# zraorg/ZRA

Measured on AMD Instinct MI355X. Metric: compress + RA-decompress GiB/s, 16 GiB @ 64 KiB frames, 1/2/4/8 MI355X, higher is better.
Workload: dtype u8

## Files before the change

zra_amd/csrc/zra_decode.hip:

```cpp
#include "zra_dev.h"
#include "zra_kernels.h"

using namespace zra_dev;

namespace {

constexpr int DEC_THREADS = 64;
constexpr int BATCH = 64;
#ifndef ZRA_XWIN
#define ZRA_XWIN 4032
#endif
constexpr u32 XPRE = 64, XWIN = ZRA_XWIN;
constexpr u32 BLOCK_MAX = 128u << 10;

__constant__ u32 c_ll_base[36] = {0,1,2,3,4,5,6,7,8,9,10,11,12,13,14,15,16,18,20,22,24,28,32,40,48,64,128,256,512,1024,2048,4096,8192,16384,32768,65536};
__constant__ u8 c_ll_bits[36] = {0,0,0,0,0,0,0,0,0,0,0,0,0,0,0,0,1,1,1,1,2,2,3,3,4,6,7,8,9,10,11,12,13,14,15,16};
__constant__ u32 c_ml_base[53] = {3,4,5,6,7,8,9,10,11,12,13,14,15,16,17,18,19,20,21,22,23,24,25,26,27,28,29,30,31,32,33,34,
                                  35,37,39,41,43,47,51,59,67,83,99,131,259,515,1027,2051,4099,8195,16387,32771,65539};
__constant__ u8 c_ml_bits[53] = {0,0,0,0,0,0,0,0,0,0,0,0,0,0,0,0,0,0,0,0,0,0,0,0,0,0,0,0,0,0,0,0,
                                 1,1,1,1,2,2,3,3,4,4,5,7,8,9,10,11,12,13,14,15,16};
__constant__ short c_ll_defnorm[36] = {4,3,2,2,2,2,2,2,2,2,2,2,2,1,1,1,2,2,2,2,2,2,2,2,2,3,2,1,1,1,1,1,-1,-1,-1,-1};
__constant__ short c_ml_defnorm[53] = {1,4,3,2,2,2,2,2,2,1,1,1,1,1,1,1,1,1,1,1,1,1,1,1,1,1,1,1,1,1,1,1,
                                       1,1,1,1,1,1,1,1,1,1,1,1,1,1,-1,-1,-1,-1,-1,-1,-1};
__constant__ short c_of_defnorm[29] = {1,1,1,1,1,1,2,2,2,1,1,1,1,1,1,1,1,1,1,1,1,1,1,1,-1,-1,-1,-1,-1};
// ... 976 lines not shown
        packed |= (e & 0xFF) << (8 * k);
        hb.skip((int)(e >> 8));
      }
      pk[g] = packed;
    }
    st128(o + i, pk[0], pk[1], pk[2], pk[3]);
  }
  for (; i + 4 <= count; i += 4) {
    hb.ensure(4 * mb);
    u32 packed = 0;
#pragma unroll
    for (int k = 0; k < 4; k++) {
      u32 e = tab[hb.peek(mb)];
      packed |= (e & 0xFF) << (8 * k);
      hb.skip((int)(e >> 8));
    }
    st32(o + i, packed);
  }
  for (; i < count; i++) { hb.ensure(mb); u32 e = tab[hb.peek(mb)]; o[i] = (u8)e; hb.skip((int)(e >> 8)); }
}

__device__ __forceinline__ bool huf_decode_stream(const ZraDecodeArgs& a, ZraDecFrame* const F, const u32 j, const u16* const tab, const u8* const w1,
                                                  const u32 strm, const u8* const lim) {
  const u32 nStreams = F->litStreams, regen = F->litRegen;
  const u32 seg = nStreams == 1 ? regen : (regen + 3) / 4;
  const u32 myLen = nStreams == 1 ? regen : (strm < 3 ? seg : regen - 3 * seg);
  u8* o = a.lits + F->litBase + (size_t)strm * seg;
  const u8* const blk = a.body + a.frameOff[frame_of(a, j) * a.offStride] + F->bpos;
  const u8* const sb = blk + F->streamOff[strm]; const u32 sl = F->streamLen[strm];
  const int mb = (int)F->hufMaxBits;
#ifndef ZRA_HUF_READER_AHEAD
#define ZRA_HUF_READER_AHEAD 1
#endif
#if ZRA_HUF_READER_AHEAD
  BitRS hb;
#else
  BitR hb;
#endif
  bool bad = hb.init(sb, sl, lim) != 0;
  if (!bad) {
    u32 i = 0;
    if (mb < 12) {
      huf_x1_emit(hb, tab, mb, o, myLen);
      i = myLen;
    } else {
      for (; i < myLen; i++) { hb.ensure(12); const u32 e = huf_lookup12(tab, w1, hb.peek(12), 12); o[i] = (u8)e; hb.skip((int)(e >> 8)); }
    }
    if (hb.pos != 0) bad = true;
  }
  if (bad && F->hufX2) bad = !huf_stream_x2(tab, w1, (u32)mb, sb, sl, lim, o, myLen);
  return !bad;
}

__device__ __forceinline__ bool huf_decode_wave(const ZraDecodeArgs& a, const ZraDecFrame* const F, const u32 j, const u16* const tab, const int lane, const u8* const lim) {
  const u32 nStreams = F->litStreams, regen = F->litRegen;
  const int mb = (int)F->hufMaxBits;
  if (mb >= 12 || regen < 64) return false;
  const u32 L = nStreams == 1 ? 64u : 16u;
  const u32 strm = nStreams == 1 ? 0u : (u32)lane >> 4, t = (u32)lane & (L - 1);
  const u32 seg = nStreams == 1 ? regen : (regen + 3) / 4;
  const u32 myLen = nStreams == 1 ? regen : (strm < 3 ? seg : regen - 3 * seg);
  const u8* const blk = a.body + a.frameOff[frame_of(a, j) * a.offStride] + F->bpos;
  const u8* const sb = blk + F->streamOff[strm]; const u32 sl = F->streamLen[strm];
  const u32 last = sl ? (u32)sb[sl - 1] : 0u;
  if (__ballot(last == 0)) return false;
  const u32 P = (sl - 1) * 8 + hb32(last);
  const u32 C = max((P + L - 1) / L, 128u);
  const bool active = t * C < P;
  const i32 lower = (t + 1) * C >= P ? 0 : (i32)(P - (t + 1) * C);
  i32 start = (i32)(P - t * C), end = 0;
  u32 n = 0;
  bool dirty = active;
  BitRS hb;
  i32 prevStart = start;
  for (int it = 0; it < 6 && __ballot(dirty); it++) {
    if (dirty) {
      bool merged = false;
      if (it) {
        BitRS ho;
        hb.init_at(sb, lim, start); ho.init_at(sb, lim, prevStart);
        u32 ka = 0, kb = 0;
        for (int k = 0; k < 96; k++) {
          if (hb.pos == ho.pos) { merged = true; break; }
          if (hb.pos <= lower || ho.pos <= lower) break;
          if (hb.pos > ho.pos) { hb.ensure(mb); const u32 e = tab[hb.peek(mb)]; hb.skip((int)(e >> 8)); ka++; }
          else { ho.ensure(mb); const u32 e = tab[ho.peek(mb)]; ho.skip((int)(e >> 8)); kb++; }
        }
        if (merged) n = ka + (n - kb);
      }
      if (!merged) {
        hb.init_at(sb, lim, start); n = 0;
        while (hb.pos > lower) {
          hb.ensure(4 * mb);
#pragma unroll
          for (int k = 0; k < 4; k++) if (hb.pos > lower) { const u32 e = tab[hb.peek(mb)]; hb.skip((int)(e >> 8)); n++; }
        }
        end = hb.pos;
      }
    }
    const i32 handed = (i32)__shfl_up(end, 1, 64);
    const i32 ns = t == 0 ? (i32)P : handed;
    prevStart = start;
    dirty = active && ns != start;
    start = ns;
#ifdef ZRA_SMALL_PROFILE
    { const u64 dm = __ballot(dirty); if (lane == 0) atomicAdd(&zra_small_prof[16 + it], (u64)__popcll(dm)); }
#endif
  }
#ifdef ZRA_SMALL_PROFILE
  if (lane == 0) atomicAdd(&zra_small_prof[6], 1ull);
  if (__ballot(dirty) && lane == 0) atomicAdd(&zra_small_prof[7], 1ull);
#endif
  if (__ballot(dirty)) return false;
  u32 incl = active ? n : 0u;
  if (L == 64) incl = dpp_scan_add(incl);
  else {
    incl += (u32)__builtin_amdgcn_update_dpp(0, (int)incl, 0x111, 0xF, 0xF, true);
    incl += (u32)__builtin_amdgcn_update_dpp(0, (int)incl, 0x112, 0xF, 0xF, true);
    incl += (u32)__builtin_amdgcn_update_dpp(0, (int)incl, 0x114, 0xF, 0xF, true);
    incl += (u32)__builtin_amdgcn_update_dpp(0, (int)incl, 0x118, 0xF, 0xF, true);
  }
  const u32 total = (u32)__shfl((int)incl, (int)(((u32)lane & ~(L - 1)) + L - 1), 64);
  if (__ballot(total != myLen || (active && lower == 0 && end != 0))) return false;
  if (active && n) {
    hb.init_at(sb, lim, start);
    huf_x1_emit(hb, tab, mb, a.lits + F->litBase + (size_t)strm * seg + (incl - n), n);
  }
  return true;
}
}

extern "C" __global__ void __launch_bounds__(DEC_THREADS)
zra_dec_huf_kernel(ZraDecodeArgs a) {
  __shared__ HufShared S;
  const int lane = threadIdx.x;
  const u32 nJobs = a.counters[ZRA_DC_NHUF];
  const u8* const lim = a.body + a.bodySize;
  for (;;) {
    wsync();
    if (lane == 0) S.base = atomicAdd(&a.counters[ZRA_DC_QHUF], (u32)HUF_FRAMES);
    wsync();
    const u32 base = S.base;
    if (base >= nJobs) return;
    const u32 nHere = min((u32)HUF_FRAMES, nJobs - base);
    for (u32 s = 0; s < nHere; s++) huf_build_table(&a.frames[a.hufJobs[base + s]], S.tab[s], S.w1[s], lane);
    wsync();
    u32 doneMask = 0;
    for (u32 s = 0; s < nHere; s++) {
      const u32 j = a.hufJobs[base + s];
      if (huf_decode_wave(a, &a.frames[j], j, S.tab[s], lane, lim)) doneMask |= 1u << s;
    }
    const u32 slot = (u32)lane >> 2, strm = (u32)lane & 3;
    if (slot < nHere && !((doneMask >> slot) & 1u)) {
      const u32 j = a.hufJobs[base + slot];
      ZraDecFrame* const F = &a.frames[j];
      if (strm < F->litStreams && !huf_decode_stream(a, F, j, S.tab[slot], S.w1[slot], strm, lim)) F->hufErr = 1;
    }
  }
}

namespace {

constexpr u32 CHAIN_RING = 128, CHAIN_RING_WORDS = (CHAIN_RING + 16) / 4;
static_assert(CHAIN_RING_WORDS == ZRA_CHAIN_RING_WORDS, "ring size: zra_kernels.h");
__device__ __attribute__((noinline)) uint4 chain_ld128_tail(const u8* p, const u8* lim) {
  u32 w[4] = {0, 0, 0, 0};
  for (u32 k = 0; k < 16; k++) if (p + k < lim) w[k >> 2] |= (u32)p[k] << (8 * (k & 3));
  return make_uint4(w[0], w[1], w[2], w[3]);
}
template <bool RING>
struct ZdsT {
  u64 c; u32 bc; u32 ptr;
  const u8* base;
  u8* ring; u32 rLo; const u8* lim; uint4 pf; u32 pfState, pfAge;
  enum : int { UNFINISHED = 0, ENDOFBUFFER = 1, COMPLETED = 2, OVERFLOW = 3 };
  __device__ __forceinline__ uint4 ld16(const u8* p) const {
    if (p + 16 <= lim) { const u128_u q = *(const u128_u*)p; return make_uint4(q.a, q.b, q.c, q.d); }
    return chain_ld128_tail(p, lim);
  }
  __device__ __forceinline__ void ring_write(u32 off, uint4 q) {
    const u32 o = off & (CHAIN_RING - 1);
    lds_st128(ring + o, q);
    if (o == 0) lds_st64(ring + CHAIN_RING, (u64)q.x | ((u64)q.y << 32));
  }
  __device__ __forceinline__ void ring_resync(u32 p) {
    const u32 pc = p & ~15u, lo = pc >= 48 ? pc - 48 : 0u;
    uint4 q[5];
#pragma unroll
    for (u32 k = 0; k < 5; k++) q[k] = ld16(base + lo + 16 * k);
#pragma unroll
    for (u32 k = 0; k < 5; k++) ring_write(lo + 16 * k, q[k]);
    rLo = lo; pfState = 0;
  }
  __device__ __forceinline__ void ring_advance() {
    if (pfState) {
      if (++pfAge >= 2 && ptr + 8 + 16 <= rLo + CHAIN_RING) { ring_write(rLo - 16, pf); rLo -= 16; pfState = 0; }
    } else if (rLo >= 16 && ptr < rLo + 64) { pf = ld16(base + rLo - 16); pfState = 1; pfAge = 0; }
  }
  __device__ __forceinline__ u64 fetch(u32 p) {
    if (RING) return *(const zra_lds_u64u_t*)(ring + (p & (CHAIN_RING - 1)));
    return ld64(base + p);
  }
  __device__ __forceinline__ void ring_guard() { if (rLo && ptr < rLo + 16) ring_resync(ptr); }
// ... 890 lines not shown
```

zra_amd/csrc/zra_dev.h:

```cpp
#pragma once
#include <hip/hip_runtime.h>
#include <stdint.h>

namespace zra_dev {

typedef uint8_t u8;
typedef uint16_t u16;
typedef uint32_t u32;
typedef uint64_t u64;
typedef int32_t i32;

enum : u32 {
  ZE_OK = 0, ZE_GENERIC = 1, ZE_PREFIX_UNKNOWN = 10, ZE_FRAMEPARAM_UNSUPPORTED = 14, ZE_WINDOW_TOO_LARGE = 16,
  ZE_CORRUPTION = 20, ZE_CHECKSUM_WRONG = 22, ZE_DICT_CORRUPTED = 30, ZE_DICT_WRONG = 32, ZE_PARAM_UNSUPPORTED = 40,
  ZE_DSTSIZE_TOOSMALL = 70, ZE_SRCSIZE_WRONG = 72,
};

constexpr int WAVE = 64;

__host__ __device__ __forceinline__ u64 frame_expect(u64 i, u64 frameSize, u64 total) {
  const u64 o = i * frameSize;
  return o >= total ? 0 : (total - o < frameSize ? total - o : frameSize);
}

__device__ __forceinline__ u32 hb32(u32 x) { return 31u - (u32)__builtin_clz(x); }
__device__ __forceinline__ int lane_id() { return (int)(threadIdx.x & 63); }

typedef u16 __attribute__((aligned(1))) u16_u;
typedef u32 __attribute__((aligned(1))) u32_u;
typedef u64 __attribute__((aligned(1))) u64_u;
__device__ __forceinline__ u32 ld16(const u8* p) { return *(const u16_u*)p; }
__device__ __forceinline__ u32 ld24(const u8* p) { return (u32)p[0] | ((u32)p[1] << 8) | ((u32)p[2] << 16); }
__device__ __forceinline__ u32 ld32(const u8* p) { return *(const u32_u*)p; }
__device__ __forceinline__ u64 ld64(const u8* p) { return *(const u64_u*)p; }
__device__ __forceinline__ u64 ld64_safe(const u8* p, const u8* end) {
  if (p + 8 <= end) return ld64(p);
  u64 v = 0;
  for (int i = 0; i < 8; i++) if (p + i < end) v |= (u64)p[i] << (8 * i);
  return v;
}
typedef __attribute__((address_space(3))) u64_u zra_lds_u64u_t;
typedef u32 zra_v4u32_t __attribute__((ext_vector_type(4)));
typedef __attribute__((address_space(3))) zra_v4u32_t zra_lds_v4u32_t;
typedef __attribute__((address_space(3))) u64 zra_lds_u64_t;
__device__ __forceinline__ void lds_st128(u8* p, uint4 q) { zra_v4u32_t v = {q.x, q.y, q.z, q.w}; *(zra_lds_v4u32_t*)p = v; }
__device__ __forceinline__ void lds_st64(u8* p, u64 v) { *(zra_lds_u64_t*)p = v; }
__device__ __forceinline__ void st32(u8* p, u32 v) { *(u32_u*)p = v; }
__device__ __forceinline__ void st64(u8* p, u64 v) { *(u64_u*)p = v; }
__device__ __forceinline__ void copy_bytes(u8* dst, const u8* src, u32 n, int t, int nthreads) {
  u32 n8 = n >> 3;
  for (u32 i = t; i < n8; i += nthreads) st64(dst + 8 * i, ld64(src + 8 * i));
  for (u32 i = (n8 << 3) + t; i < n; i += nthreads) dst[i] = src[i];
}
__device__ __forceinline__ void copy_slice(u8* dst, const u8* src, u32 n, int lane) {
  if ((((uintptr_t)dst ^ (uintptr_t)src) & 15u) || n < 64) { copy_bytes(dst, src, n, lane, 64); return; }
  const u32 head = (u32)((16u - ((uintptr_t)dst & 15u)) & 15u);
  if ((u32)lane < head) dst[lane] = src[lane];
  const u32 n16 = (n - head) >> 4;
  const uint4* s4 = (const uint4*)(src + head);
  uint4* d4 = (uint4*)(dst + head);
  for (u32 i = lane; i < n16; i += 64) d4[i] = s4[i];
  for (u32 i = head + (n16 << 4) + lane; i < n; i += 64) dst[i] = src[i];
}
__device__ __forceinline__ u64 seek_entry(const u8* table, u64 f) { const u8* e = table + (size_t)f * 5; return (u64)ld32(e) | ((u64)e[4] << 32); }
struct Slice { u32 tuple; u64 frame; u32 inFrame; u32 len; u64 user; };
__device__ __forceinline__ Slice slice_of(const u64* q, u32 nq, u64 s, u64 fs) {
  u32 lo = 0, hi = nq - 1;
  while (lo < hi) {
    const u32 mid = lo + (hi - lo + 1) / 2;
    if (q[4 * (size_t)mid + 3] <= s) lo = mid; else hi = mid - 1;
  }
  const u64 off = q[4 * (size_t)lo], size = q[4 * (size_t)lo + 1], k = s - q[4 * (size_t)lo + 3];
  const u64 f0 = off / fs, head = off - f0 * fs;
  Slice r;
  r.tuple = lo; r.frame = f0 + k;
  r.inFrame = k ? 0u : (u32)head;
  const u64 done = k ? (fs - head) + (k - 1) * fs : 0;
  r.len = (u32)min<u64>(fs - r.inFrame, size - done);
  r.user = q[4 * (size_t)lo + 2] + done;
  return r;
}
struct __attribute__((packed, aligned(1))) u128_u { u32 a, b, c, d; };
__device__ __forceinline__ void st128(u8* p, u32 a, u32 b, u32 c, u32 d) { u128_u v; v.a = a; v.b = b; v.c = c; v.d = d; *(u128_u*)p = v; }

__device__ __forceinline__ u32 wave_incl_scan(u32 v) {
  int l = lane_id();
#pragma unroll
  for (int d = 1; d < 64; d <<= 1) {
    u32 t = __shfl_up(v, d, 64);
    if (l >= d) v += t;
  }
  return v;
}
__device__ __forceinline__ u32 wave_sum(u32 v) {
#pragma unroll
  for (int d = 32; d > 0; d >>= 1) v += __shfl_xor(v, d, 64);
  return v;
}
__device__ __forceinline__ u32 wave_max(u32 v) {
#pragma unroll
  for (int d = 32; d > 0; d >>= 1) { u32 t = __shfl_xor(v, d, 64); v = t > v ? t : v; }
  return v;
}

struct BitR {
  const u8* base;
  const u8* lim;
  i32 pos;
  i32 wlo;
  u64 w;
  __device__ __forceinline__ void reload() {
    i32 byteIdx = ((pos + 7) >> 3) - 8;
    if (byteIdx >= 0) { w = ld64_safe(base + byteIdx, lim); wlo = byteIdx * 8; }
    else {
      i32 sh = -byteIdx * 8;
      w = sh >= 64 ? 0 : (ld64_safe(base, lim) << sh);
      wlo = byteIdx * 8;
    }
  }
  __device__ __forceinline__ int init(const u8* b, u32 n, const u8* bufLim) {
    base = b; lim = bufLim;
    if (n == 0) return 1;
    u32 last = b[n - 1];
    if (last == 0) return 1;
    pos = (i32)(n - 1) * 8 + (i32)hb32(last);
    reload();
    return 0;
  }
  __device__ __forceinline__ void ensure(int nb) { if (pos - wlo < nb) reload(); }
  __device__ __forceinline__ u32 peek(int nb) const {
    return (u32)((w >> (pos - nb - wlo)) & ((1ull << nb) - 1));
  }
  __device__ __forceinline__ void skip(int nb) { pos -= nb; }
  __device__ __forceinline__ u32 read(int nb) {
    if (nb == 0) return 0;
    ensure(nb);
    u32 v = peek(nb);
    pos -= nb;
    return v;
  }
};

struct BitRS {
  const u8* base; const u8* lim;
  i32 pos, wlo; u64 w;
  i32 gtop;
  u64 g0, g1, g2;
  __device__ __forceinline__ u64 grid(i32 idx) const {
    if (idx >= 0) return ld64_safe(base + idx, lim);
    if (idx <= -8) return 0;
    return ld64_safe(base, lim) << (u32)(-idx * 8);
  }
  __device__ __forceinline__ void reload() {
    const i32 byteIdx = ((pos + 7) >> 3) - 8;
    while (byteIdx <= gtop - 8) { g0 = g1; g1 = g2; gtop -= 8; g2 = grid(gtop - 16); }
    const u32 d = (u32)(gtop - byteIdx);
    w = d ? ((g0 << (8 * d)) | (g1 >> (64 - 8 * d))) : g0;
    wlo = byteIdx * 8;
  }
  __device__ __forceinline__ int init(const u8* b, u32 n, const u8* bufLim) {
    base = b; lim = bufLim;
    if (n == 0) return 1;
    u32 last = b[n - 1];
    if (last == 0) return 1;
    pos = (i32)(n - 1) * 8 + (i32)hb32(last);
    gtop = ((pos + 7) >> 3) - 8;
    g0 = grid(gtop); g1 = grid(gtop - 8); g2 = grid(gtop - 16);
    w = g0; wlo = gtop * 8;
    return 0;
  }
  __device__ __forceinline__ void init_at(const u8* b, const u8* bufLim, i32 p) {
    base = b; lim = bufLim; pos = p;
    gtop = ((pos + 7) >> 3) - 8;
    g0 = grid(gtop); g1 = grid(gtop - 8); g2 = grid(gtop - 16);
    w = g0; wlo = gtop * 8;
  }
  __device__ __forceinline__ void ensure(int nb) { if (pos - wlo < nb) reload(); }
  __device__ __forceinline__ u32 peek(int nb) const { return (u32)((w >> (pos - nb - wlo)) & ((1ull << nb) - 1)); }
  __device__ __forceinline__ void skip(int nb) { pos -= nb; }
};


constexpr u64 XP1 = 11400714785074694791ULL, XP2 = 14029467366897019727ULL, XP3 = 1609587929392839161ULL,
              XP4 = 9650029242287828579ULL, XP5 = 2870177450012600261ULL;
__device__ __forceinline__ u64 rotl64(u64 x, int r) { return (x << r) | (x >> (64 - r)); }
__device__ __forceinline__ u64 xxround(u64 acc, u64 x) { return rotl64(acc + x * XP2, 31) * XP1; }
__device__ __forceinline__ u64 xxmerge(u64 h, u64 v) { return (h ^ xxround(0, v)) * XP1 + XP4; }


__device__ inline u64 zra_xxh64_quad(const u8* p, u32 n, int j) {
  u64 v = j == 0 ? XP1 + XP2 : j == 1 ? XP2 : j == 2 ? 0 : (0 - XP1);
  const u32 stripes = n >> 5;
  const u8* q = p + 8 * j;
  u32 s = 0;
  for (; s + 8 <= stripes; s += 8) {
    u64 x[8];
#pragma unroll
    for (int k = 0; k < 8; k++) x[k] = ld64(q + 32 * (size_t)(s + k));
#pragma unroll
    for (int k = 0; k < 8; k++) v = xxround(v, x[k]);
  }
  for (; s < stripes; s++) v = xxround(v, ld64(q + 32 * (size_t)s));
  const int base = (threadIdx.x & 63) & ~3;
  u64 v1 = __shfl(v, base + 0, 64), v2 = __shfl(v, base + 1, 64), v3 = __shfl(v, base + 2, 64), v4 = __shfl(v, base + 3, 64);
  u64 h;
  if (n >= 32) {
    h = rotl64(v1, 1) + rotl64(v2, 7) + rotl64(v3, 12) + rotl64(v4, 18);
    h = xxmerge(h, v1); h = xxmerge(h, v2); h = xxmerge(h, v3); h = xxmerge(h, v4);
  } else h = XP5;
  h += (u64)n;
  if (j == 0) {
    const u8* t = p + ((size_t)stripes << 5); u32 rem = n & 31;
    while (rem >= 8) { h = rotl64(h ^ xxround(0, ld64(t)), 27) * XP1 + XP4; t += 8; rem -= 8; }
    if (rem >= 4) { h = rotl64(h ^ ((u64)ld32(t) * XP1), 23) * XP2 + XP3; t += 4; rem -= 4; }
    while (rem) { h = rotl64(h ^ ((u64)*t * XP5), 11) * XP1; t++; rem--; }
    h ^= h >> 33; h *= XP2; h ^= h >> 29; h *= XP3; h ^= h >> 32;
  }
  return h;
}

__device__ inline u64 zra_xxh64_quad_seed(const u8* p, u64 n, int j, u64 seed) {
  u64 v = seed + (j == 0 ? XP1 + XP2 : j == 1 ? XP2 : j == 2 ? 0 : (0 - XP1));
  const u64 stripes = n >> 5;
  const u8* q = p + 8 * j;
  u64 s = 0;
  for (; s + 8 <= stripes; s += 8) {
    u64 x[8];
#pragma unroll
    for (int k = 0; k < 8; k++) x[k] = ld64(q + 32 * (size_t)(s + k));
#pragma unroll
    for (int k = 0; k < 8; k++) v = xxround(v, x[k]);
  }
// ... 22 lines not shown
```

zra_amd/csrc/zra_engine.h:

```cpp
#pragma once
#include <hip/hip_runtime.h>
#include <cstdint>
#include <cstddef>
#include <vector>
#include "zra_kernels.h"
#include "zra_scan_plan.h"

namespace zra_eng {

struct Status { int zra; int zstd; };
enum : int { kSuccess = 0, kZStdError = 1, kVersionLow = 2, kHeaderInvalid = 3, kHeaderIncomplete = 4, kOutOfBounds = 5,
             kOutputTooSmall = 6, kCompressedTooLarge = 7, kFrameSizeMismatch = 8 };
inline Status ok() { return {kSuccess, 0}; }
inline Status zerr(int code) { return {kZStdError, (int)(int8_t)code}; }

struct DevBuf {
  void* p = nullptr; size_t cap = 0;
  bool reserve(size_t n);
  void release();
  template <typename T> T* as() const { return (T*)p; }
};

uint64_t scratch_bytes_in_use();

// ... 147 lines not shown
  void locate_records_stats(uint64_t out[8]) const { for (int i = 0; i < 8; i++) out[i] = lstats_[i]; }
  double locate_records_ms() const { return locateMs_; }
  Status read_records(const uint8_t* dArc, size_t arcSize, const uint64_t info6[6], const uint64_t* dIndex, size_t indexWords, const uint64_t* hNumbers, size_t n,
                      size_t stagingBytes, uint64_t* hRanges, uint8_t* dData, size_t dataCap, uint64_t* dataSize);
  void read_records_stats(uint64_t out[8]) const { for (int i = 0; i < 8; i++) out[i] = rstats_[i]; }
  double read_records_ms() const { return readMs_; }

  Status compress_host(const uint8_t* hIn, size_t n, uint8_t* hOut, size_t* outSize, int level, uint32_t frameSize, bool checksum);
  Status compress_frames_host(const uint8_t* hIn, size_t n, uint8_t* hBody, std::vector<uint64_t>& sizes, size_t* bodySize,
                              int level, uint32_t frameSize, bool checksum);
  Status decode_host(const uint8_t* hSpan, size_t spanSize, const std::vector<uint64_t>& starts, const std::vector<uint64_t>& ends,
                     uint32_t frameSize, uint64_t total, uint8_t* hOut, size_t skip, size_t size, bool wholeArchive = false);
  Status decode_host_pipelined(const uint8_t* hSpan, const std::vector<uint64_t>& starts, const std::vector<uint64_t>& ends,
                               uint32_t frameSize, uint64_t total, uint8_t* hOut, bool* fallBack);

  void set_ra_verify_whole_frames(bool on) { raVerifyWholeFrames_ = on; }
  bool ra_verify_whole_frames() const { return raVerifyWholeFrames_; }
  int device() const { return device_; }
  int num_cus() const { return numCUs_; }

 private:
  Engine() = default;
  int device_ = 0, numCUs_ = 0;
  hipStream_t stream_ = nullptr;
  hipEvent_t ev0_ = nullptr, ev1_ = nullptr, evWait_ = nullptr;
  double lastKernelMs_ = 0;
  std::vector<uint64_t> mfTele_;
  const uint64_t* mfTeleDev_ = nullptr;
  double kstats_[6] = {0, 0, 0, 0, 0, 0};
  double dstats_[8] = {0, 0, 0, 0, 0, 0, 0, 0};
  std::vector<hipEvent_t> stageEv_; size_t stageEvNext_ = 0;
  hipEvent_t stage_event();
  Status launch_stages(uint64_t nJobs, const struct ZraDecodeArgs& a, const struct ZraDecodeArgs& mid, uint32_t nFrames, bool blockPass, hipEvent_t se[5]);
  Status launch_chain(uint64_t nJobs, const struct ZraDecodeArgs& mid, hipEvent_t after);
  Status decode_sequential_tail(const struct ZraDecodeArgs& a, const uint64_t* dFrameOff, uint32_t offStride, const uint64_t* dOutOff, uint32_t first,
                                uint32_t nFrames, uint32_t maxFrameBytes, uint64_t seqTotal);
  Status upload_jobs(const std::vector<uint64_t>& frameOff, const std::vector<uint64_t>& outOff, const std::vector<uint32_t>& expect);
  Status read_fixed_header(const uint8_t* dArc, size_t arcSize, HeaderInfo* h);
  uint64_t* pinned_tuples(size_t nTuples);
  void reset_decode_stats() { kstats_[4] = kstats_[5] = 0; for (auto& d : dstats_) d = 0; }
  static float elapsed_ms(hipEvent_t e0, hipEvent_t e1) { float ms = 0; if (hipEventElapsedTime(&ms, e0, e1) != hipSuccess) { ms = 0; (void)hipGetLastError(); } return ms; }
  bool call_events() {
    for (auto& ev : evCall_) if (!ev && hipEventCreate(&ev) != hipSuccess) { ev = nullptr; (void)hipGetLastError(); return false; }
    return true;
  }
  void free_scratch();
  hipEvent_t evR_[17] = {nullptr};
  DevBuf decFrames_, decTables_, decLists_, decCounters_, decLits_, decSeqs_, roundN_;
  DevBuf decBlkRecs_, decBlkTables_, decBlkLists_;
  DevBuf raPlan_, raLimit_, raPieceBase_, raPieces_;
  uint8_t* pinSmall_ = nullptr;
  uint64_t* pinQ_ = nullptr; size_t pinQCap_ = 0;
  int decOccParse_ = 0, decOccExec_ = 0, decOccHuf_ = 0;
  bool raVerifyWholeFrames_ = false;
  DevBuf status_, produced_, frameMeta_, frameOff_, outOff_, expect_, result_, qmeta_;
  DevBuf stage_;
  struct EncCtx { DevBuf tables, seqs, lits, work, slots, misc, ck, sizes, rec; };
  EncCtx encCtx_[2];
  DevBuf encScan_;
  DevBuf mfFlags_;
  int lsAttr_ = 0;
  hipStream_t stream2_ = nullptr;
  bool decCountersClean_ = false;
  int chainLdsAttr_ = 0;
  hipStream_t pipeStreams_[2] = {nullptr, nullptr};
  std::vector<hipEvent_t> evPool_;
  DevBuf hostIn_, hostOut_, seqScratch_;
  uint64_t dbgSeqStride_ = 0; uint32_t dbgB_ = 0;
  uint64_t lastProducedTotal_ = ~0ull;
  void* encCounters_ = nullptr; size_t encCountersBytes_ = 0;
  int waitValueOk_ = 0;
  struct UpdScratch { DevBuf plan, packed, encSizes, frames, table, copies; } upd_;
  uint64_t ustats_[8] = {0, 0, 0, 0, 0, 0, 0, 0};
  hipEvent_t evCall_[2] = {nullptr, nullptr};
  double updStageMs_ = 0;
  struct VerifyScratch { DevBuf plan, faults; } vfy_;
  uint64_t vstats_[8] = {0, 0, 0, 0, 0, 0, 0, 0};
  struct ScanScratch { DevBuf tables, list; } scan_;
  uint64_t scanStats_[kScanCalls][8] = {};
  double scanMs_[kScanCalls] = {};
  struct CompareScratch { DevBuf flags, tables, list; } cmp_;
  uint64_t cstats_[8] = {0, 0, 0, 0, 0, 0, 0, 0}, cmpSizes_[2] = {0, 0};
  double compareMs_ = 0;
  uint64_t fstats_[8] = {0, 0, 0, 0, 0, 0, 0, 0};
  double diffMs_ = 0;
  struct SignScratch { DevBuf flags, dirty, tables, list; } sig_;
  uint64_t gstats_[8] = {0, 0, 0, 0, 0, 0, 0, 0}, hstats_[8] = {0, 0, 0, 0, 0, 0, 0, 0};
  double signMs_ = 0, sigDiffMs_ = 0;
  struct RecScratch { DevBuf tables, ranges; } rec_;
  uint64_t istats_[8] = {0, 0, 0, 0, 0, 0, 0, 0}, lstats_[8] = {0, 0, 0, 0, 0, 0, 0, 0}, rstats_[8] = {0, 0, 0, 0, 0, 0, 0, 0};
  double indexMs_ = 0, locateMs_ = 0, readMs_ = 0;
  friend struct EncodeImpl;
  friend struct UpdateImpl;
  friend struct VerifyImpl;
  friend struct ScanImpl;
  friend struct CompareImpl;
  friend struct DiffImpl;
  friend struct SignImpl;
  friend struct RecordsImpl;
  friend class ArchiveCache;
};

void search_launch_jobs(hipStream_t s, const uint8_t* table, uint64_t fs, uint64_t total, uint64_t first, uint32_t n, uint64_t* frameOff, uint64_t* outOff,
                        uint32_t* expect);
void search_launch_scan(hipStream_t s, const uint32_t* counts, uint32_t nItems, uint64_t* bases, const uint64_t* cntIn, uint64_t* cntOut);
void search_launch_carry(hipStream_t s, uint8_t* win, uint64_t L, uint32_t n);
// ... 5 lines not shown
```

zra_amd/csrc/zra_engine.hip:

```cpp
#include "zra_host.h"
#include "zra_dev.h"
#include "zra_format.h"
#include <algorithm>
#include <atomic>

extern "C" __global__ void zra_dec_parse_kernel(ZraDecodeArgs a);
extern "C" __global__ void zra_dec_huf_kernel(ZraDecodeArgs a);
extern "C" __global__ void zra_dec_chain_kernel(ZraDecodeArgs a);
extern "C" __global__ void zra_dec_chain_lds_kernel(ZraDecodeArgs a);
extern "C" __global__ void zra_dec_exec_kernel(ZraDecodeArgs a);
extern "C" __global__ void zra_dec_parse_all_kernel(ZraDecodeArgs a);
extern "C" __global__ void zra_dec_exec_all_kernel(ZraDecodeArgs a);
extern "C" __global__ void zra_ra_small_kernel(ZraDecodeArgs a, uint32_t* bail, const uint32_t* expect, uint32_t jobBase, unsigned long long* result);

using namespace zra_dev;

namespace zra_fmt {
uint32_t crc32(uint32_t crc, const void* data, size_t n) {
  static uint32_t T[8][256];
  static bool init = false;
  if (!init) {
    for (uint32_t i = 0; i < 256; i++) {
      uint32_t c = i;
      for (int k = 0; k < 8; k++) c = (c & 1) ? (0xEDB88320u ^ (c >> 1)) : (c >> 1);
// ... 192 lines not shown
  HIPCHK(hipMemcpyAsync(two, result_.p, 16, hipMemcpyDeviceToHost, stream_));
  trace.mark("queued rest");
  HIPCHK(hipStreamSynchronize(stream_));
  trace.mark("sync");
  HIPCHK(hipGetLastError());
  if (hipMemsetAsync(a.counters, 0, ZRA_DC_WORDS * 4, stream_) == hipSuccess) decCountersClean_ = true;
  two[1] = 0xFFFFFFFFull - (two[1] & 0xFFFFFFFFull);
  *bailed = (uint32_t)two[1];
  if (!*bailed) *hResult = two[0];
  float ms = 0;
  if (hipEventElapsedTime(&ms, ev0_, ev1_) == hipSuccess) { lastKernelMs_ = ms; kstats_[4] += ms; kstats_[5] += 1; dstats_[5] += ms; dstats_[6] += 1; }
  return ok();
}

hipEvent_t Engine::stage_event() {
  if (stageEvNext_ == stageEv_.size()) { hipEvent_t e = nullptr; if (hipEventCreate(&e) != hipSuccess) return nullptr; stageEv_.push_back(e); }
  return stageEv_[stageEvNext_++];
}

Status Engine::launch_chain(uint64_t nJobs, const ZraDecodeArgs& mid, hipEvent_t after) {
  constexpr uint32_t chainWaves = 2;
  static const uint32_t chainLdsMin = (uint32_t)zra_env::env_int("ZRA_DEC_CHAIN_LDS_MIN", numCUs_ * 96);
  static const int chainLdsMode = zra_env::env_int("ZRA_DEC_CHAIN_LDS", 1);
  const uint32_t gridChain = (uint32_t)std::min<uint64_t>((nJobs + 63) / 64, (uint64_t)numCUs_ * chainWaves);
  if (chainLdsMode != 0 && nJobs >= chainLdsMin) {
    if (!pipeStreams_[1]) { if (hipStreamCreateWithFlags(&pipeStreams_[1], hipStreamNonBlocking) != hipSuccess) { pipeStreams_[1] = nullptr; (void)hipGetLastError(); } }
    const size_t ldsBytes = (128 + (size_t)ZRA_CHAIN_LDS_FRAMES * (ZRA_DEC_TBL_WORDS / 2 + ZRA_CHAIN_RING_WORDS)) * 4;
    if (pipeStreams_[1] && !chainLdsAttr_) {
      if (hipFuncSetAttribute((const void*)zra_dec_chain_lds_kernel, hipFuncAttributeMaxDynamicSharedMemorySize, (int)ldsBytes) == hipSuccess) chainLdsAttr_ = 1;
      else { chainLdsAttr_ = -1; (void)hipGetLastError(); }
    }
    if (pipeStreams_[1] && chainLdsAttr_ > 0) {
      hipEvent_t eJoin = stage_event(); if (!eJoin) return zerr(1);
      HIPCHK(hipStreamWaitEvent(pipeStreams_[1], after, 0));
      hipLaunchKernelGGL(zra_dec_chain_lds_kernel, dim3((uint32_t)numCUs_), dim3(64), ldsBytes, pipeStreams_[1], mid);
      HIPCHK(hipEventRecord(eJoin, pipeStreams_[1]));
      if (chainLdsMode != 2) hipLaunchKernelGGL(zra_dec_chain_kernel, dim3(gridChain), dim3(64), 0, stream_, mid);
      HIPCHK(hipStreamWaitEvent(stream_, eJoin, 0));
      return ok();
    }
  }
  hipLaunchKernelGGL(zra_dec_chain_kernel, dim3(gridChain), dim3(64), 0, stream_, mid);
  return ok();
}

Status Engine::launch_stages(uint64_t nJobs, const ZraDecodeArgs& a, const ZraDecodeArgs& mid, uint32_t nFrames, bool blockPass, hipEvent_t se[5]) {
  for (int k = 0; k < 5; k++) { se[k] = stage_event(); if (!se[k]) return zerr(1); }
  const uint32_t gridParse = (uint32_t)std::min<uint64_t>(nFrames, (uint64_t)numCUs_ * decOccParse_);
  const uint32_t gridHuf = (uint32_t)std::min<uint64_t>((nJobs + ZRA_HUF_FRAMES - 1) / ZRA_HUF_FRAMES, (uint64_t)numCUs_ * decOccHuf_);
  const uint32_t gridExec = (uint32_t)std::min<uint64_t>(nFrames, (uint64_t)numCUs_ * decOccExec_);
  HIPCHK(hipEventRecord(se[0], stream_));
  hipLaunchKernelGGL(blockPass ? zra_dec_parse_all_kernel : zra_dec_parse_kernel, dim3(gridParse), dim3(64), 0, stream_, a);
  HIPCHK(hipEventRecord(se[1], stream_));
  hipLaunchKernelGGL(zra_dec_huf_kernel, dim3(gridHuf), dim3(64), 0, stream_, mid);
  HIPCHK(hipEventRecord(se[2], stream_));
  { Status st = launch_chain(nJobs, mid, se[2]); if (st.zra) return st; }
  HIPCHK(hipEventRecord(se[3], stream_));
  hipLaunchKernelGGL(blockPass ? zra_dec_exec_all_kernel : zra_dec_exec_kernel, dim3(gridExec), dim3(64), 0, stream_, a);
  HIPCHK(hipEventRecord(se[4], stream_));
  return ok();
}

Status Engine::decode_launch(const ZraDecodeArgs& a0, const uint32_t* dExpect, uint32_t maxFrameBytes, uint32_t jobBase, unsigned long long* hResult) {
  ZraDecodeArgs a = a0;
  const uint32_t n = a.nFrames;
  { Status st = decode_scratch(a, maxFrameBytes); if (st.zra) return st; }
  decCountersClean_ = false;
  uint32_t* listA = decLists_.as<uint32_t>(); uint32_t* listB = listA + n;
  if (!decOccParse_) {
    HIPCHK(hipOccupancyMaxActiveBlocksPerMultiprocessor(&decOccParse_, zra_dec_parse_kernel, 64, 0));
    HIPCHK(hipOccupancyMaxActiveBlocksPerMultiprocessor(&decOccExec_, zra_dec_exec_kernel, 64, 0));
    HIPCHK(hipOccupancyMaxActiveBlocksPerMultiprocessor(&decOccHuf_, zra_dec_huf_kernel, 64, 0));
    decOccParse_ = std::max(1, decOccParse_); decOccExec_ = std::max(1, decOccExec_); decOccHuf_ = std::max(1, decOccHuf_);
  }
  HIPCHK(hipEventRecord(ev0_, stream_));
  constexpr uint32_t aheadCap = 16;
  if (!roundN_.reserve(4 * (aheadCap + 2) + 64)) return zerr(64);
  static const int fmbEnv = zra_env::env_int("ZRA_DEC_FMB", 1);
  static const uint32_t fmbMin = (uint32_t)zra_env::env_int("ZRA_DEC_FMB_MIN", 64);
  const uint32_t bpf = (uint32_t)(((uint64_t)maxFrameBytes + ZRA_FMB_BLOCK - 1) / ZRA_FMB_BLOCK);
  bool fmb = fmbEnv != 0 && bpf >= 2 && maxFrameBytes <= (64u << 20) && n >= fmbMin && (uint64_t)n * bpf < (1ull << 30);
  uint32_t nRest = n;
  if (fmb) {
    const uint64_t nb = (uint64_t)n * bpf;
    const uint64_t litAll = std::max<uint64_t>((uint64_t)n * ((uint64_t)maxFrameBytes + 16) / 2, 1u << 20);
    const uint64_t seqAll = std::max<uint64_t>((uint64_t)n * ((uint64_t)maxFrameBytes + 16) * 3 / 32, 1u << 20);
    if (!decBlkRecs_.reserve((size_t)nb * sizeof(ZraDecFrame)) || !decBlkTables_.reserve((size_t)nb * ZRA_DEC_TBL_WORDS * 4) ||
        !decBlkLists_.reserve((size_t)(2 * nb + n) * 4 + 64) || !decLits_.reserve(litAll + 64) || !decSeqs_.reserve(seqAll * 8 + 64)) {
      (void)hipGetLastError();
      fmb = false;
    }
    a.lits = decLits_.as<uint8_t>(); a.seqs = decSeqs_.as<uint64_t>();
    if (fmb) {
      ZraDecodeArgs x = a;
      x.bpf = bpf; x.blkRecs = decBlkRecs_.as<ZraDecFrame>(); x.blkTables = decBlkTables_.as<uint32_t>();
      uint32_t* bl = decBlkLists_.as<uint32_t>();
      x.pending = bl; x.hufJobs = bl + nb; x.execList = bl + 2 * nb;
      x.litCap = litAll; x.seqCap = seqAll;
      x.active = nullptr; x.nActive = n; x.round = 0; x.nActivePtr = nullptr; x.nextActive = listA;
      HIPCHK(hipMemsetAsync(x.counters, 0, ZRA_DC_WORDS * 4, stream_));
      ZraDecodeArgs y = x; y.frames = x.blkRecs; y.tables = x.blkTables;
      hipEvent_t se[5];
      { Status st = launch_stages(nb, x, y, n, true, se); if (st.zra) return st; }
      uint32_t back = 0;
      HIPCHK(hipMemcpyAsync(&back, x.counters + ZRA_DC_NNEXT, 4, hipMemcpyDeviceToHost, stream_));
      HIPCHK(hipStreamSynchronize(stream_));
      HIPCHK(hipGetLastError());
      for (int k = 0; k < 4; k++) { float m = 0; if (hipEventElapsedTime(&m, se[k], se[k + 1]) == hipSuccess) dstats_[k] += m; }
      dstats_[4] += 1;
      stageEvNext_ = 0;
      nRest = back;
    }
  }
  auto run_rounds = [&](ZraDecodeArgs& x, uint32_t nActive, const uint32_t* active, uint32_t round, uint32_t* lA, uint32_t* lB, uint32_t ahead) -> Status {
    uint32_t* const dN = roundN_.as<uint32_t>();
    while (nActive) {
      const uint32_t burst = std::max(1u, std::min(ahead, aheadCap));
      hipEvent_t se[aheadCap][5];
      for (uint32_t bi = 0; bi < burst; bi++) {
        HIPCHK(hipMemsetAsync(x.counters, 0, ZRA_DC_WORDS * 4, stream_));
        x.active = active; x.nActive = nActive; x.round = round + bi;
        x.nActivePtr = bi ? dN + bi : nullptr;
        x.nextActive = (active == lA) ? lB : lA;
        { Status st = launch_stages(nActive, x, x, nActive, false, se[bi]); if (st.zra) return st; }
        HIPCHK(hipMemcpyAsync(dN + bi + 1, x.counters + ZRA_DC_NNEXT, 4, hipMemcpyDeviceToDevice, stream_));
// ... 198 lines not shown
```

zra_amd/csrc/zra_kernels.h:

```cpp
#pragma once
#include <stdint.h>
#include <stddef.h>

#ifndef ZRA_HUF_FRAMES
#define ZRA_HUF_FRAMES 2
#endif
#define ZRA_DEC_TBL_LL 0u
#define ZRA_DEC_TBL_ML 512u
#define ZRA_DEC_TBL_OF 1024u
#define ZRA_DEC_TBL_WORDS 1280u
#define ZRA_LDS_TBL_LL 0u
#define ZRA_LDS_TBL_ML 1024u
#define ZRA_LDS_TBL_OF 2048u
#define ZRA_LDS_TBL_WORDS 2304u
#define ZRA_CHAIN_LDS_FRAMES 59u
#define ZRA_CHAIN_RING_WORDS 36u

struct ZraDecFrame {
  uint32_t blkPos, produced, done;
  uint32_t hufValid, hufMaxBits, hufNSym, hufX2;
  uint32_t llValid, mlValid, ofValid, llLog, mlLog, ofLog, ofShare;
  uint32_t rep[3];
  uint32_t fcsLo, fcsHi, fcsHave, hasChecksum, bigWindow;
  uint32_t bpos, bsize, blast;
  uint32_t litKind, litRegen, litArg;
  uint32_t litStreams, streamOff[4], streamLen[4];
  uint32_t hufErr, lateErr;
  uint32_t nbSeq, seqPos, longMode;
  uint64_t litBase, seqBase;
  uint32_t chainErr, nSeqValid, seqOut, seqLit, truncated;
  uint32_t repOut[3];
  uint32_t nBlk, endPos, parseTrunc, pad1_;
  alignas(8) uint8_t weights[256];
  alignas(8) uint16_t hufStart[256];
};
#define ZRA_REP_MARK_LO 0x0C000000u
#define ZRA_REP_MARK(k) (ZRA_REP_MARK_LO + ((uint32_t)(k) << 24) + 0x00800000u)
#define ZRA_FMB_BLOCK (128u << 10)

struct ZraRaPiece { uint64_t dstOff; uint32_t srcOff, len; };

struct RaPlan {
  uint32_t* cnt;
  uint32_t* need;
  uint32_t* slot;
  uint32_t* cursor;
  uint32_t* totals;
  static constexpr size_t kTotalsWords = 16;
  static size_t words(uint32_t nFrames) { return 4 * (size_t)nFrames + kTotalsWords; }
  static RaPlan over(uint32_t* p, uint32_t n) { return RaPlan{p, p + n, p + 2 * (size_t)n, p + 3 * (size_t)n, p + 4 * (size_t)n}; }
  uint32_t* lookup_words() const { return totals + 8; }
};

struct ZraDecodeArgs {
  const uint8_t* body;
  uint64_t bodySize;
  const uint64_t* frameOff;
  uint32_t offStride;
  uint8_t* out;
  const uint64_t* outOff;
  const uint32_t* outCap;
  uint32_t nFrames;
  const uint32_t* limit;
  const uint32_t* pieceBase;
  const ZraRaPiece* pieces;
  uint8_t* raOut;
  const uint32_t* active;
  uint32_t nActive;
  const uint32_t* nActivePtr;
  uint32_t round;
  uint32_t* counters;
  uint32_t* nextActive;
  uint32_t* pending;
  uint32_t* hufJobs;
  ZraDecFrame* frames;
  uint32_t* tables;
  uint8_t* lits; uint64_t litCap;
  uint64_t* seqs; uint64_t seqCap;
  uint32_t* status;
  uint32_t* produced;
  uint32_t* frameMeta;
  uint32_t debugSkip;
  uint32_t bpf;
  ZraDecFrame* blkRecs;
  uint32_t* blkTables;
  uint32_t* execList;
};
#define ZRA_DC_QPARSE 0
#define ZRA_DC_QCHAIN 1
#define ZRA_DC_QEXEC 2
#define ZRA_DC_NPENDING 3
#define ZRA_DC_NNEXT 4
#define ZRA_DC_NHUF 5
#define ZRA_DC_QHUF 10
#define ZRA_DC_LITCUR 6
#define ZRA_DC_SEQCUR 8
#define ZRA_DC_NEXEC 11
#define ZRA_DC_QEXECALL 12
#define ZRA_DC_WORDS 16

struct ZraEncParams {
  uint32_t windowLog, chainLog, hashLog, searchLog, minMatch, targetLength, strategy;
  uint32_t blockSize;
};

#define ZRA_OPT_NUM 4096u
struct ZraOptCell { int32_t price; uint32_t off, mlen, litlen, rep[3]; };
struct ZraOptMatch { uint32_t off, len; };
struct ZraOptState {
  uint32_t litFreq[256], litLengthFreq[36], matchLengthFreq[53], offCodeFreq[32];
  uint32_t litSum, litLengthSum, matchLengthSum, offCodeSum;
  uint32_t litSumBasePrice, litLengthSumBasePrice, matchLengthSumBasePrice, offCodeSumBasePrice;
  uint32_t predef, pad;
  ZraOptCell table[ZRA_OPT_NUM + 1];
  ZraOptMatch matches[ZRA_OPT_NUM + 1];
};

struct ZraFseCTable {
  uint16_t stateTable[512];
  uint32_t deltaNbBits[53];
  int32_t deltaFindState[53];
  uint32_t tableLog, maxSym, rle;
};

struct alignas(16) ZraEncFrameState {
  uint32_t rep[3];
  uint32_t nextToUpdate;
  uint32_t insEnd;
  uint32_t pad0_[3];
  uint32_t ring[128][4];
  uint32_t idxShift;
  uint32_t outPos;
  uint32_t hufRepeat;
  uint32_t llRepeat, ofRepeat, mlRepeat;
  uint32_t hufMaxSym;
// ... 85 lines not shown
```

Measured before the change: 20.64.

## Stage Huffman literal streams into LDS before wave-parallel decode

Adds a dynamic-LDS staging buffer (8 KiB by default) into which each wave copies the compressed Huffman stream bytes with 128-bit loads before the speculative parallel decode. The bit reader is templated over its source so the same decode loop reads from LDS instead of bounds-checked global loads. When the whole block does not fit, streams are staged and decoded one at a time, and jobs that still exceed the buffer fall back to global memory. HUF_FRAMES drops from 2 to 1, likely to offset the LDS cost. This trades repeated scattered global reads during resync and emit passes for an upfront copy, extra LDS pressure and possibly lower occupancy.

Result: faster. 20.87 (median of 4 runs) (+1.1%).

```diff
diff --git a/zra_amd/csrc/zra_decode.hip b/zra_amd/csrc/zra_decode.hip
--- a/zra_amd/csrc/zra_decode.hip
+++ b/zra_amd/csrc/zra_decode.hip
@@ -1052,17 +1052,14 @@
   return !bad;
 }
 
-__device__ __forceinline__ bool huf_decode_wave(const ZraDecodeArgs& a, const ZraDecFrame* const F, const u32 j, const u16* const tab, const int lane, const u8* const lim) {
+template <typename Src>
+__device__ __forceinline__ bool huf_wave_runs(const ZraDecodeArgs& a, const ZraDecFrame* const F, const u16* const tab, const int lane,
+                                              const Src& src, const u32 sl, const u32 last, const u32 strm, const u32 L) {
   const u32 nStreams = F->litStreams, regen = F->litRegen;
   const int mb = (int)F->hufMaxBits;
-  if (mb >= 12 || regen < 64) return false;
-  const u32 L = nStreams == 1 ? 64u : 16u;
-  const u32 strm = nStreams == 1 ? 0u : (u32)lane >> 4, t = (u32)lane & (L - 1);
+  const u32 t = (u32)lane & (L - 1);
   const u32 seg = nStreams == 1 ? regen : (regen + 3) / 4;
   const u32 myLen = nStreams == 1 ? regen : (strm < 3 ? seg : regen - 3 * seg);
-  const u8* const blk = a.body + a.frameOff[frame_of(a, j) * a.offStride] + F->bpos;
-  const u8* const sb = blk + F->streamOff[strm]; const u32 sl = F->streamLen[strm];
-  const u32 last = sl ? (u32)sb[sl - 1] : 0u;
   if (__ballot(last == 0)) return false;
   const u32 P = (sl - 1) * 8 + hb32(last);
   const u32 C = max((P + L - 1) / L, 128u);
@@ -1071,14 +1068,14 @@
   i32 start = (i32)(P - t * C), end = 0;
   u32 n = 0;
   bool dirty = active;
-  BitRS hb;
+  BitRSx<Src> hb;
   i32 prevStart = start;
   for (int it = 0; it < 6 && __ballot(dirty); it++) {
     if (dirty) {
       bool merged = false;
       if (it) {
-        BitRS ho;
-        hb.init_at(sb, lim, start); ho.init_at(sb, lim, prevStart);
+        BitRSx<Src> ho;
+        hb.init_at(src, start); ho.init_at(src, prevStart);
         u32 ka = 0, kb = 0;
         for (int k = 0; k < 96; k++) {
           if (hb.pos == ho.pos) { merged = true; break; }
@@ -1089,7 +1086,7 @@
         if (merged) n = ka + (n - kb);
       }
       if (!merged) {
-        hb.init_at(sb, lim, start); n = 0;
+        hb.init_at(src, start); n = 0;
         while (hb.pos > lower) {
           hb.ensure(4 * mb);
 #pragma unroll
@@ -1123,19 +1120,75 @@
   const u32 total = (u32)__shfl((int)incl, (int)(((u32)lane & ~(L - 1)) + L - 1), 64);
   if (__ballot(total != myLen || (active && lower == 0 && end != 0))) return false;
   if (active && n) {
-    hb.init_at(sb, lim, start);
+    hb.init_at(src, start);
     huf_x1_emit(hb, tab, mb, a.lits + F->litBase + (size_t)strm * seg + (incl - n), n);
   }
   return true;
 }
-}
-
+__device__ __forceinline__ bool huf_decode_wave(const ZraDecodeArgs& a, const ZraDecFrame* const F, const u32 j, const u16* const tab, const int lane, const u8* const lim) {
+  const u32 nStreams = F->litStreams;
+  if (F->hufMaxBits >= 12 || F->litRegen < 64) return false;
+  const u32 L = nStreams == 1 ? 64u : 16u;
+  const u32 strm = nStreams == 1 ? 0u : (u32)lane >> 4;
+  const u8* const blk = a.body + a.frameOff[frame_of(a, j) * a.offStride] + F->bpos;
+  const u8* const sb = blk + F->streamOff[strm]; const u32 sl = F->streamLen[strm];
+  const u32 last = sl ? (u32)sb[sl - 1] : 0u;
+  return huf_wave_runs(a, F, tab, lane, StreamMem{sb, lim}, sl, last, strm, L);
+}
+
+__device__ __forceinline__ u32 huf_stage_bytes(const u8* const g, const u32 n, const u32 stage, const int lane) {
+  wsync();
+  const u32 mis = (u32)((uintptr_t)g & 15u);
+  const u32 head = min(n, (16u - mis) & 15u);
+  const u32 dst = stage + mis;
+  if ((u32)lane < head) *(zra_lds_u8_t*)(dst + (u32)lane) = g[lane];
+  const u32 n16 = (n - head) >> 4;
+  const uint4* const g16 = (const uint4*)(g + head);
+  const u32 d16 = dst + head;
+  u32 i = (u32)lane;
+  for (; i + 192 < n16; i += 256) {
+    const uint4 v0 = g16[i], v1 = g16[i + 64], v2 = g16[i + 128], v3 = g16[i + 192];
+    lds_st128_at(d16 + 16 * i, v0); lds_st128_at(d16 + 16 * (i + 64), v1);
+    lds_st128_at(d16 + 16 * (i + 128), v2); lds_st128_at(d16 + 16 * (i + 192), v3);
+  }
+  for (; i < n16; i += 64) lds_st128_at(d16 + 16 * i, g16[i]);
+  const u32 tail = head + (n16 << 4) + (u32)lane;
+  if (tail < n) *(zra_lds_u8_t*)(dst + tail) = g[tail];
+  wsync();
+  return dst;
+}
+__device__ __forceinline__ bool huf_decode_job(const ZraDecodeArgs& a, const ZraDecFrame* const F, const u32 j, const u16* const tab, const int lane, const u8* const lim,
+                                               const u32 stage, const u32 cap) {
+  const u32 nStreams = F->litStreams;
+  if (F->hufMaxBits >= 12 || F->litRegen < 64) return false;
+  const u32 off0 = F->streamOff[0], bytes = F->streamOff[nStreams - 1] + F->streamLen[nStreams - 1] - off0;
+  const bool whole = cap && bytes <= cap;
+  bool each = false;
+  if (cap && !whole && nStreams == 4) each = max(max(F->streamLen[0], F->streamLen[1]), max(F->streamLen[2], F->streamLen[3])) <= cap;
+  if (!whole && !each) return huf_decode_wave(a, F, j, tab, lane, lim);
+  const u8* const blk = a.body + a.frameOff[frame_of(a, j) * a.offStride] + F->bpos;
+  const u32 passes = each ? 4u : 1u;
+  for (u32 p = 0; p < passes; p++) {
+    const u32 L = (each || nStreams == 1) ? 64u : 16u;
+    const u32 strm = each ? p : (nStreams == 1 ? 0u : (u32)lane >> 4);
+    const u32 first = each ? F->streamOff[p] : off0;
+    const u32 base = huf_stage_bytes(blk + first, each ? F->streamLen[p] : bytes, stage, lane);
+    const u32 so = base + (F->streamOff[strm] - first), sl = F->streamLen[strm];
+    const u32 last = sl ? (u32)*(const zra_lds_u8_t*)(so + sl - 1) : 0u;
+    if (!huf_wave_runs(a, F, tab, lane, StreamLds{so}, sl, last, strm, L)) return false;
+  }
+  return true;
+}
+}
+
+extern __shared__ __attribute__((aligned(16))) u8 hufStageLds[];
 extern "C" __global__ void __launch_bounds__(DEC_THREADS)
 zra_dec_huf_kernel(ZraDecodeArgs a) {
   __shared__ HufShared S;
   const int lane = threadIdx.x;
   const u32 nJobs = a.counters[ZRA_DC_NHUF];
   const u8* const lim = a.body + a.bodySize;
+  const u32 stage = (u32)(uintptr_t)(zra_lds_u8_t*)hufStageLds, cap = a.hufStage;
   for (;;) {
     wsync();
     if (lane == 0) S.base = atomicAdd(&a.counters[ZRA_DC_QHUF], (u32)HUF_FRAMES);
@@ -1148,7 +1201,7 @@
     u32 doneMask = 0;
     for (u32 s = 0; s < nHere; s++) {
       const u32 j = a.hufJobs[base + s];
-      if (huf_decode_wave(a, &a.frames[j], j, S.tab[s], lane, lim)) doneMask |= 1u << s;
+      if (huf_decode_job(a, &a.frames[j], j, S.tab[s], lane, lim, stage, cap)) doneMask |= 1u << s;
     }
     const u32 slot = (u32)lane >> 2, strm = (u32)lane & 3;
     if (slot < nHere && !((doneMask >> slot) & 1u)) {
diff --git a/zra_amd/csrc/zra_dev.h b/zra_amd/csrc/zra_dev.h
--- a/zra_amd/csrc/zra_dev.h
+++ b/zra_amd/csrc/zra_dev.h
@@ -43,7 +43,9 @@
 typedef u32 zra_v4u32_t __attribute__((ext_vector_type(4)));
 typedef __attribute__((address_space(3))) zra_v4u32_t zra_lds_v4u32_t;
 typedef __attribute__((address_space(3))) u64 zra_lds_u64_t;
+typedef __attribute__((address_space(3))) u8 zra_lds_u8_t;
 __device__ __forceinline__ void lds_st128(u8* p, uint4 q) { zra_v4u32_t v = {q.x, q.y, q.z, q.w}; *(zra_lds_v4u32_t*)p = v; }
+__device__ __forceinline__ void lds_st128_at(u32 addr, uint4 q) { zra_v4u32_t v = {q.x, q.y, q.z, q.w}; *(zra_lds_v4u32_t*)addr = v; }
 __device__ __forceinline__ void lds_st64(u8* p, u64 v) { *(zra_lds_u64_t*)p = v; }
 __device__ __forceinline__ void st32(u8* p, u32 v) { *(u32_u*)p = v; }
 __device__ __forceinline__ void st64(u8* p, u64 v) { *(u64_u*)p = v; }
@@ -141,15 +143,24 @@
   }
 };
 
-struct BitRS {
+struct StreamMem {
   const u8* base; const u8* lim;
+  __device__ __forceinline__ u64 ld8(i32 idx) const { return ld64_safe(base + idx, lim); }
+};
+struct StreamLds {
+  u32 base;
+  __device__ __forceinline__ u64 ld8(i32 idx) const { return *(const zra_lds_u64u_t*)(base + (u32)idx); }
+};
+template <typename Src>
+struct BitRSx {
+  Src src;
   i32 pos, wlo; u64 w;
   i32 gtop;
   u64 g0, g1, g2;
   __device__ __forceinline__ u64 grid(i32 idx) const {
-    if (idx >= 0) return ld64_safe(base + idx, lim);
+    if (idx >= 0) return src.ld8(idx);
     if (idx <= -8) return 0;
-    return ld64_safe(base, lim) << (u32)(-idx * 8);
+    return src.ld8(0) << (u32)(-idx * 8);
   }
   __device__ __forceinline__ void reload() {
     const i32 byteIdx = ((pos + 7) >> 3) - 8;
@@ -158,26 +169,25 @@
     w = d ? ((g0 << (8 * d)) | (g1 >> (64 - 8 * d))) : g0;
     wlo = byteIdx * 8;
   }
+  __device__ __forceinline__ void init_at(const Src& s, i32 p) {
+    src = s; pos = p;
+    gtop = ((pos + 7) >> 3) - 8;
+    g0 = grid(gtop); g1 = grid(gtop - 8); g2 = grid(gtop - 16);
+    w = g0; wlo = gtop * 8;
+  }
+  __device__ __forceinline__ void ensure(int nb) { if (pos - wlo < nb) reload(); }
+  __device__ __forceinline__ u32 peek(int nb) const { return (u32)((w >> (pos - nb - wlo)) & ((1ull << nb) - 1)); }
+  __device__ __forceinline__ void skip(int nb) { pos -= nb; }
+};
+struct BitRS : BitRSx<StreamMem> {
   __device__ __forceinline__ int init(const u8* b, u32 n, const u8* bufLim) {
-    base = b; lim = bufLim;
     if (n == 0) return 1;
     u32 last = b[n - 1];
     if (last == 0) return 1;
-    pos = (i32)(n - 1) * 8 + (i32)hb32(last);
-    gtop = ((pos + 7) >> 3) - 8;
-    g0 = grid(gtop); g1 = grid(gtop - 8); g2 = grid(gtop - 16);
-    w = g0; wlo = gtop * 8;
+    BitRSx<StreamMem>::init_at(StreamMem{b, bufLim}, (i32)(n - 1) * 8 + (i32)hb32(last));
     return 0;
   }
-  __device__ __forceinline__ void init_at(const u8* b, const u8* bufLim, i32 p) {
-    base = b; lim = bufLim; pos = p;
-    gtop = ((pos + 7) >> 3) - 8;
-    g0 = grid(gtop); g1 = grid(gtop - 8); g2 = grid(gtop - 16);
-    w = g0; wlo = gtop * 8;
-  }
-  __device__ __forceinline__ void ensure(int nb) { if (pos - wlo < nb) reload(); }
-  __device__ __forceinline__ u32 peek(int nb) const { return (u32)((w >> (pos - nb - wlo)) & ((1ull << nb) - 1)); }
-  __device__ __forceinline__ void skip(int nb) { pos -= nb; }
+  __device__ __forceinline__ void init_at(const u8* b, const u8* bufLim, i32 p) { BitRSx<StreamMem>::init_at(StreamMem{b, bufLim}, p); }
 };
 
 
diff --git a/zra_amd/csrc/zra_engine.h b/zra_amd/csrc/zra_engine.h
--- a/zra_amd/csrc/zra_engine.h
+++ b/zra_amd/csrc/zra_engine.h
@@ -223,6 +223,7 @@
   uint8_t* pinSmall_ = nullptr;
   uint64_t* pinQ_ = nullptr; size_t pinQCap_ = 0;
   int decOccParse_ = 0, decOccExec_ = 0, decOccHuf_ = 0;
+  uint32_t decHufStage_ = 0;
   bool raVerifyWholeFrames_ = false;
   DevBuf status_, produced_, frameMeta_, frameOff_, outOff_, expect_, result_, qmeta_;
   DevBuf stage_;
diff --git a/zra_amd/csrc/zra_engine.hip b/zra_amd/csrc/zra_engine.hip
--- a/zra_amd/csrc/zra_engine.hip
+++ b/zra_amd/csrc/zra_engine.hip
@@ -268,7 +268,9 @@
   HIPCHK(hipEventRecord(se[0], stream_));
   hipLaunchKernelGGL(blockPass ? zra_dec_parse_all_kernel : zra_dec_parse_kernel, dim3(gridParse), dim3(64), 0, stream_, a);
   HIPCHK(hipEventRecord(se[1], stream_));
-  hipLaunchKernelGGL(zra_dec_huf_kernel, dim3(gridHuf), dim3(64), 0, stream_, mid);
+  ZraDecodeArgs huf = mid;
+  huf.hufStage = decHufStage_;
+  hipLaunchKernelGGL(zra_dec_huf_kernel, dim3(gridHuf), dim3(64), decHufStage_ ? decHufStage_ + ZRA_HUF_STAGE_PAD : 0, stream_, huf);
   HIPCHK(hipEventRecord(se[2], stream_));
   { Status st = launch_chain(nJobs, mid, se[2]); if (st.zra) return st; }
   HIPCHK(hipEventRecord(se[3], stream_));
@@ -286,7 +288,9 @@
   if (!decOccParse_) {
     HIPCHK(hipOccupancyMaxActiveBlocksPerMultiprocessor(&decOccParse_, zra_dec_parse_kernel, 64, 0));
     HIPCHK(hipOccupancyMaxActiveBlocksPerMultiprocessor(&decOccExec_, zra_dec_exec_kernel, 64, 0));
-    HIPCHK(hipOccupancyMaxActiveBlocksPerMultiprocessor(&decOccHuf_, zra_dec_huf_kernel, 64, 0));
+    decHufStage_ = (uint32_t)std::min(std::max(zra_env::env_int("ZRA_DEC_HUF_STAGE", ZRA_HUF_STAGE_BYTES), 0), 96 << 10);
+    if (decHufStage_ && hipFuncSetAttribute((const void*)zra_dec_huf_kernel, hipFuncAttributeMaxDynamicSharedMemorySize, (int)(decHufStage_ + ZRA_HUF_STAGE_PAD)) != hipSuccess) { decHufStage_ = 0; (void)hipGetLastError(); }
+    HIPCHK(hipOccupancyMaxActiveBlocksPerMultiprocessor(&decOccHuf_, zra_dec_huf_kernel, 64, decHufStage_ ? decHufStage_ + ZRA_HUF_STAGE_PAD : 0));
     decOccParse_ = std::max(1, decOccParse_); decOccExec_ = std::max(1, decOccExec_); decOccHuf_ = std::max(1, decOccHuf_);
   }
   HIPCHK(hipEventRecord(ev0_, stream_));
diff --git a/zra_amd/csrc/zra_kernels.h b/zra_amd/csrc/zra_kernels.h
--- a/zra_amd/csrc/zra_kernels.h
+++ b/zra_amd/csrc/zra_kernels.h
@@ -3,8 +3,12 @@
 #include <stddef.h>
 
 #ifndef ZRA_HUF_FRAMES
-#define ZRA_HUF_FRAMES 2
+#define ZRA_HUF_FRAMES 1
 #endif
+#ifndef ZRA_HUF_STAGE_BYTES
+#define ZRA_HUF_STAGE_BYTES 8192
+#endif
+#define ZRA_HUF_STAGE_PAD 32u
 #define ZRA_DEC_TBL_LL 0u
 #define ZRA_DEC_TBL_ML 512u
 #define ZRA_DEC_TBL_OF 1024u
@@ -80,7 +84,7 @@
   uint32_t* status;
   uint32_t* produced;
   uint32_t* frameMeta;
-  uint32_t debugSkip;
+  uint32_t hufStage;
   uint32_t bpf;
   ZraDecFrame* blkRecs;
   uint32_t* blkTables;
```
